# lvclark/tagdigger

Hardware: NVIDIA B200
Metric: reads/sec (whole box), 200M-read 96-plex GBS FASTQ (higher is better)
Workload: dtype u8 text -> 2-bit keys, int32 counts

## Files before the change

### tagdigger_b200/csrc/tdg_kernel.cuh

```cuda
#pragma once
#include <cuda_runtime.h>
#include <stdint.h>
#include <stddef.h>
#include "tdg_match.h"

namespace tdg {

#ifndef TDG_WARPS
#define TDG_WARPS 14
#endif
#ifndef TDG_CHUNKS
#define TDG_CHUNKS 15
#endif
#ifndef TDG_HALO
#define TDG_HALO 256
#endif

constexpr int      WARPS = TDG_WARPS;
constexpr int      THREADS = WARPS * 32;
constexpr uint32_t CHUNKS = TDG_CHUNKS;
constexpr uint32_t SPAN = CHUNKS * 16;
constexpr uint32_t MWORDS = (SPAN + 31) / 32;
constexpr uint32_t HALF_WORDS = MWORDS / 2;
constexpr uint32_t TILE = 32 * SPAN;
// ... 73 lines not shown
    unsigned long long *totals;
};

struct VerifyArgs {
    uint32_t num_segs;
    uint32_t use_arg_state;
    uint32_t prev_kind;
    uint32_t make_fixes;
    unsigned long long line_base;
    unsigned long long reads_limit;
    const LineState *state_in;
    LineState *state_out;
    const SegInfo *seginfo;
    const uint32_t *last_kind;
    FixEntry *fix;
    uint32_t *n_fix;
    unsigned long long *run_total;
};

inline uint32_t fast_words_for(const BarTable *bar, const TagTable &tt)
{
    if (bar->any_base || tt.any_base) return 0;
    if (bar->max_len > 16 || bar->max_tag_off > 28) return 0;
    if (tt.n_classes != 1 || tt.max_len > 64 + LONG_TAIL_MAX || tt.min_len < 1) return 0;
    uint32_t chars = 3 + bar->max_tag_off + tt.max_len;
    if (chars < 3 + 16) chars = 3 + 16;
    uint32_t nw = (chars + 3) / 4;
    return nw <= (tt.max_len > 64 ? LONG_WORDS_MAX : FAST_WORDS_MAX) ? nw : 0;
}
inline bool fast_is_long(const TagTable &tt) { return tt.max_len > 64; }

#if defined(__CUDACC__)

struct alignas(16) WarpShared {
    uint16_t q[QCAP];
    uint16_t gs[GUESS_LINES + 8];
};
static_assert(sizeof(WarpShared) % 16 == 0, "control blocks must keep the barcode table 16-byte aligned");

constexpr size_t SMEM_FIXED = (size_t)WARPS * RING + (size_t)WARPS * sizeof(WarpShared);

__device__ __forceinline__ uint32_t smem_u32(const void *p)
{
    return (uint32_t)__cvta_generic_to_shared(p);
}
__device__ __forceinline__ void mbar_init(uint64_t *bar, uint32_t count)
{
    asm volatile("mbarrier.init.shared::cta.b64 [%0], %1;" ::"r"(smem_u32(bar)), "r"(count));
}
__device__ __forceinline__ void mbar_expect_tx(uint64_t *bar, uint32_t bytes)
{
    asm volatile("mbarrier.arrive.expect_tx.shared::cta.b64 _, [%0], %1;" ::"r"(smem_u32(bar)), "r"(bytes)
                 : "memory");
}
__device__ __forceinline__ void mbar_wait(uint64_t *bar, uint32_t parity)
{
    asm volatile(
        "{\n"
        ".reg .pred p;\n"
        "WAIT_%=:\n"
        "mbarrier.try_wait.parity.shared::cta.b64 p, [%0], %1;\n"
        "@p bra DONE_%=;\n"
        "bra WAIT_%=;\n"
        "DONE_%=:\n"
        "}\n" ::"r"(smem_u32(bar)),
        "r"(parity)
        : "memory");
}
__device__ __forceinline__ bool mbar_test(uint64_t *bar, uint32_t parity)
{
    uint32_t ok;
    asm volatile(
        "{\n"
        ".reg .pred p;\n"
        "mbarrier.try_wait.parity.shared::cta.b64 p, [%1], %2;\n"
        "selp.u32 %0, 1, 0, p;\n"
        "}\n"
        : "=r"(ok)
        : "r"(smem_u32(bar)), "r"(parity)
        : "memory");
    return ok != 0;
}
__device__ __forceinline__ void bulk_g2s(void *dst, const void *src, uint32_t bytes, uint64_t *bar)
{
    uint64_t policy;
    asm volatile("createpolicy.fractional.L2::evict_first.b64 %0, 1.0;" : "=l"(policy));
    asm volatile(
        "cp.async.bulk.shared::cluster.global.mbarrier::complete_tx::bytes.L2::cache_hint [%0], [%1], %2, [%3], %4;" ::"r"(
            smem_u32(dst)),
        "l"(src), "r"(bytes), "r"(smem_u32(bar)), "l"(policy)
        : "memory");
}

__device__ __forceinline__ uint32_t notctl4(uint32_t w)
{
    uint32_t r;
    asm("prmt.b32 %0, %1, %2, %3;" : "=r"(r) : "r"(w + 0x60606060u), "r"(0u), "r"(0xBA98u));
    return r;
}
__device__ __forceinline__ int32_t dp4a_su(uint32_t a_signed_bytes, uint32_t b_unsigned_bytes, int32_t c)
{
    int32_t d;
    asm("dp4a.s32.u32 %0, %1, %2, %3;" : "=r"(d) : "r"(a_signed_bytes), "r"(b_unsigned_bytes), "r"(c));
    return d;
}
__device__ __forceinline__ uint32_t ctl_mask16(uint4 q, uint32_t &dev)
{
    const uint32_t nx = notctl4(q.x), ny = notctl4(q.y), nz = notctl4(q.z), nw = notctl4(q.w);
    const int32_t lo = dp4a_su(ny, 0x80402010u, dp4a_su(nx, 0x08040201u, 255));
    const int32_t hi = dp4a_su(nw, 0x80402010u, dp4a_su(nz, 0x08040201u, 255));
    dev |= ((q.x ^ 0x0A0A0A0Au) & ~nx) | ((q.y ^ 0x0A0A0A0Au) & ~ny);
    dev |= ((q.z ^ 0x0A0A0A0Au) & ~nz) | ((q.w ^ 0x0A0A0A0Au) & ~nw);
    return (uint32_t)hi * 256u + (uint32_t)lo;
}

struct SmemFetch {
    const uint8_t *p;
    uint32_t limit;
    __device__ __forceinline__ void load8(uint32_t off, uint32_t w[8]) const
    {
        const uint8_t *q = p + off;
        uint32_t sh = ((uint32_t)(uintptr_t)q & 3u) * 8u;
        const uint32_t *a = (const uint32_t *)((uintptr_t)q & ~(uintptr_t)3);
        uint32_t prev = a[0];
#pragma unroll
        for (int i = 0; i < 8; i++) {
            uint32_t nxt = a[i + 1];
            w[i] = __funnelshift_r(prev, nxt, sh);
            prev = nxt;
        }
    }
};

struct GlobalFetch {
    const uint8_t *p;
    uint32_t limit;
    __device__ __forceinline__ void load8(uint32_t off, uint32_t w[8]) const
    {
#pragma unroll 1
        for (int i = 0; i < 8; i++) {
            uint32_t v = 0;
            for (int k = 0; k < 4; k++) {
                uint32_t o = off + 4 * i + k;
                uint32_t c = o < limit ? p[o] : 0u;
                v |= c << (8 * k);
            }
            w[i] = v;
        }
    }
};

__device__ __noinline__ MatchResult match_general(const uint8_t *buf, uint32_t pos, uint32_t staged,
                                                  const uint8_t *gtile, unsigned long long avail, uint32_t need,
                                                  const BarTable *bar, const BarEntry *bent, const TagTable *tt)
{
    while (pos < staged) {
        uint32_t c = buf[pos];
        if (is_lead_space(c)) { pos++; continue; }
        if (c >= 0xC2 && c <= 0xE3 && pos + 2 < staged) {
            uint32_t u = utf8_space(c, buf[pos + 1], buf[pos + 2]);
            if (u) { pos += u; continue; }
        }
        break;
    }
    if (pos + need <= staged || staged == avail) {
        SmemFetch f;
        f.p = buf + pos;
        unsigned long long room = avail - pos;
        f.limit = room > 0x7FFFFFFFull ? 0x7FFFFFFFu : (uint32_t)room;
        return match_line(f, bar, bent, *tt);
    }
    unsigned long long gp = pos;
    while (gp < avail) {
        uint32_t c = gtile[gp];
        if (is_lead_space(c)) { gp++; continue; }
        if (c >= 0xC2 && c <= 0xE3 && gp + 2 < avail) {
            uint32_t u = utf8_space(c, gtile[gp + 1], gtile[gp + 2]);
            if (u) { gp += u; continue; }
        }
        break;
    }
    GlobalFetch f;
    f.p = gtile + gp;
    unsigned long long room = avail - gp;
    f.limit = room > 0x7FFFFFFFull ? 0x7FFFFFFFu : (uint32_t)room;
    return match_line(f, bar, bent, *tt);
}

__device__ __forceinline__ uint32_t pack_word(uint32_t w, uint32_t &bad)
{
    uint32_t c2 = (w >> 1) & 0x03030303u;
    uint32_t m = (c2 >> 1) & ~c2 & 0x01010101u;
    bad = (w & 0xD9D9D9D9u) ^ (0x41414141u ^ (m * 0x11u));
    return c2 * 0x01041040u;
}

__device__ __forceinline__ uint32_t lowmask32(uint32_t nbases)
{
    return nbases >= 16 ? 0xFFFFFFFFu : ((1u << (2 * nbases)) - 1u);
}

template <bool MATCH, bool LONG = false>
__global__ void __launch_bounds__(THREADS, 1) count_kernel(const __grid_constant__ ChunkArgs a)
{
    extern __shared__ __align__(128) uint8_t smem[];
    __shared__ __align__(8) uint64_t full_bar[WARPS][STAGES];

    constexpr uint32_t NONE = 0xFFFFFFFFu;
    constexpr uint32_t FULL = 0xFFFFFFFFu;
    const uint32_t tid = threadIdx.x;
    const uint32_t lane = tid & 31u;
    const uint32_t warp = tid >> 5;

    uint8_t *const wbase = smem + (size_t)warp * RING;
    WarpShared *const ws = (WarpShared *)(smem + (size_t)WARPS * RING) + warp;
    uint8_t *const bar_smem = smem + SMEM_FIXED;

    const uint32_t prev_kind = a.use_arg_state ? a.prev_kind : a.state_in->prev_kind;
    if ((a.mode == MODE_FIX ? *a.n_fix : a.num_segs) == 0) return;

    const BarTable *bar = a.bar;
    if (MATCH) {
        if (a.bar_in_smem) {
            const uint4 *src = (const uint4 *)a.bar;
            uint4 *dst = (uint4 *)bar_smem;
            for (uint32_t i = tid; i < (a.bar_bytes + 15u) / 16u; i += THREADS) dst[i] = src[i];
            bar = (const BarTable *)bar_smem;
        }
    }
    const BarEntry *bent = (const BarEntry *)((const uint8_t *)bar + sizeof(BarTable));
    if (lane == 0) {
        for (int s = 0; s < STAGES; s++) mbar_init(&full_bar[warp][s], 1);
        asm volatile("fence.mbarrier_init.release.cluster;" ::: "memory");
        asm volatile("fence.proxy.async.shared::cta;" ::: "memory");
    }
    __syncthreads();

    const uint32_t copy_bytes = TILE + a.halo_bytes;

    uint32_t p_item = NONE, p_seg = 0, p_tix = 0, p_ntiles = 0;
    uint32_t ticket = 0;
    if (lane == 0) ticket = atomicAdd((unsigned int *)a.ticket, 1u);
    auto produce = [&](uint32_t st, uint32_t &m_tile, uint32_t &m_item, uint32_t &m_tixf) {
        if (p_tix == p_ntiles) {
            const uint32_t n_items = a.mode == MODE_FIX ? 2u * *a.n_fix : a.num_segs;
            const uint32_t t = __shfl_sync(FULL, ticket, 0);
            p_tix = 0;
            if (t < n_items) {
                p_item = t;
                const uint32_t seg = a.mode == MODE_FIX ? a.fix[t >> 1].seg : t;
                const bool big = seg < a.n_big;
                const uint32_t want = big ? a.seg_tiles : a.seg_small;
                p_seg = big ? seg * a.seg_tiles : a.n_big * a.seg_tiles + (seg - a.n_big) * a.seg_small;
                const uint32_t left = a.num_tiles - p_seg;
                p_ntiles = left < want ? left : want;
            } else {
                p_item = NONE;
                p_ntiles = NONE;
            }
            asm volatile("" ::"r"(p_item), "r"(p_seg), "r"(p_ntiles));
        }
        m_tile = p_seg + p_tix;
        m_item = p_item;
        m_tixf = p_tix + 1 == p_ntiles ? (p_tix | TIX_LAST) : p_tix;
        if (p_item != NONE) {
            if (lane == 0) {
                const unsigned long long off = (unsigned long long)m_tile * TILE;
                uint32_t bytes = copy_bytes;
                if (__builtin_expect(m_tile + 2 >= a.num_tiles, 0)) {
                    const unsigned long long left = a.n - off;
                    if (left < bytes) bytes = ((uint32_t)left + 15u) & ~15u;
                }
                mbar_expect_tx(&full_bar[warp][st], bytes);
                bulk_g2s(wbase + st * STAGE, a.bytes + off, bytes, &full_bar[warp][st]);
            }
            p_tix++;
            if (p_tix == p_ntiles && lane == 0) ticket = atomicAdd((unsigned int *)a.ticket, 1u);
        }
    };

    const uint32_t nw = MATCH ? a.fast_words : 0;
    int32_t *wmatrix = a.matrix;
    if (MATCH && a.n_replicas > 1) {
        const uint32_t rep = (blockIdx.x * WARPS + warp) % a.n_replicas;
        if (rep) wmatrix = a.replicas + (size_t)(rep - 1) * a.cells;
    }
    const uint4 *tag_entries = (const uint4 *)a.tags.entries;
    int32_t my_bar = 0, my_tag = 0;

    uint32_t seg_lines = 0;
    uint32_t seg_reads = 0;
    uint32_t phase = 0;
    bool has_limit = false;
    int32_t weight = 1;
    bool need_guess = false;
    bool classify_first = false;

    uint32_t cur_tile = 0, cur_item = NONE, cur_tixf = 0;
    uint32_t nxt_tile[STAGES - 1], nxt_item[STAGES - 1], nxt_tixf[STAGES - 1];

    auto tag_differs = [&](const uint4 &k, uint32_t L, uint32_t T0, uint32_t T1, uint32_t T2, uint32_t T3) -> uint32_t {
        if (a.ulen) return ((k.x ^ T0) & a.um[0]) | ((k.y ^ T1) & a.um[1]) | ((k.z ^ T2) & a.um[2]) | ((k.w ^ T3) & a.um[3]);
        return ((k.x ^ T0) & lowmask32(L)) | ((k.y ^ T1) & lowmask32(L > 16 ? L - 16 : 0)) |
               ((k.z ^ T2) & lowmask32(L > 32 ? L - 32 : 0)) | ((k.w ^ T3) & lowmask32(L > 48 ? L - 48 : 0));
    };

    bool pb_pending = false;
    int32_t pb_row = -1, pb_col = -1;
    bool pb_probe = false;
    uint32_t pb_T0 = 0, pb_T1 = 0, pb_T2 = 0, pb_T3 = 0, pb_h = 0, pb_V = 0xFFFFFFFFu, pb_end = 0;
    uint4 pb_k0 = make_uint4(0, 0, 0, 0), pb_k1 = pb_k0;
    uint2 pb_m0 = make_uint2(0, 0), pb_m1 = pb_m0;
    uint32_t pb_x0 = 0, pb_x1 = 0;
    uint32_t pb_TL[LONG ? LONG_TAIL_MAX / 16 : 1];
    constexpr uint32_t NG = (LONG ? LONG_WORDS_MAX : FAST_WORDS_MAX) / 4;

    auto batch_front = [&](uint32_t qoff, uint32_t nb, uint32_t st) {
        uint32_t off = st * STAGE;
        const bool have = lane < nb;
        if (have) off = ws->q[qoff + lane];
        pb_row = -1;
        pb_col = -1;
        pb_probe = false;
        const uint32_t c0 = (*(const uint32_t *)(wbase + (off & ~3u)) >> (8u * (off & 3u))) & 0xFFu;
        const bool lead = (c0 == 0x09) | (c0 == 0x0b) | (c0 == 0x0c) | ((c0 - 0x1cu) <= 4u) | (c0 >= 0x80);
        const bool slow = have & ((nw == 0) | (cur_tile + 2 >= a.num_tiles) | lead);
        __syncwarp();
        if (nw != 0) {
            const uint32_t sh = off & 3u;
            const uint32_t *wp = (const uint32_t *)(wbase + (off & ~3u));
            uint32_t P[NG + 1];
            uint32_t GB[NG];
            auto pack_group = [&](uint32_t g) {
                uint32_t x[4], gbad = 0;
#pragma unroll
                for (uint32_t k = 0; k < 4; k++) {
                    uint32_t bad;
                    x[k] = pack_word(wp[4 * g + k], bad);
                    if (g == 0 && k == 0) bad &= 0xFFFFFFFFu << (8u * sh);
                    gbad |= bad;
                }
                GB[g] = gbad;
                P[g] = __byte_perm(__byte_perm(x[0], x[1], 0x0073), __byte_perm(x[2], x[3], 0x0073), 0x5410);
            };
#pragma unroll
            for (uint32_t g = 0; g < NG; g++) { P[g] = 0; GB[g] = 0; }
            P[NG] = 0;
            pack_group(0);
            pack_group(1);
            const uint32_t key0 = __funnelshift_r(P[0], P[1], 2u * sh);
            uint32_t tag_off = 0, blen = 0;
            int32_t row = -1;
            {
                const uint32_t b = key0 & 0xFFu;
                const uint32_t lo = bar->bucket[b], hi = bar->bucket[b + 1];
                const uint4 be0 = *(const uint4 *)(bent + lo), be1 = *(const uint4 *)(bent + lo + 1);
                const bool h0 = (lo < hi) & (((key0 ^ be0.x) & be0.y) == 0);
                const bool h1 = (lo + 1 < hi) & (((key0 ^ be1.x) & be1.y) == 0);
                uint32_t rz = h0 ? be0.z : be1.z, rw = h0 ? be0.w : be1.w;
                bool hit = h0 | h1;
                if (!hit & (lo + 2 < hi)) {
                    for (uint32_t e = lo + 2; e < hi; e++) {
                        const uint4 be = *(const uint4 *)(bent + e);
                        if (((key0 ^ be.x) & be.y) == 0) { rz = be.z; rw = be.w; hit = true; break; }
                    }
                }
                if (hit) {
                    row = (int32_t)rz;
                    blen = rw & 0xFFFFu;
                    tag_off = rw >> 16;
                }
            }
            __syncwarp();
            pack_group(2);
            pack_group(3);
            const uint32_t toff = sh + tag_off;
            const uint32_t bit = (toff & 15u) * 2u;
            const bool up = (toff >> 4) != 0;
            {
                const uint32_t Q0 = up ? P[1] : P[0], Q1 = up ? P[2] : P[1], Q2 = up ? P[3] : P[2];
                pb_T0 = __funnelshift_r(Q0, Q1, bit);
                pb_T1 = __funnelshift_r(Q1, Q2, bit);
            }
            const uint64_t pre = (((uint64_t)pb_T1 << 32) | pb_T0) & a.tag_km;
            pb_h = tag_slot(pre, a.tags.cls[0].mask);
            const bool want = have & !slow & (row >= 0);
            {
                const uint4 *e0 = tag_entries + 2 * (size_t)(a.tags.cls[0].base + (want ? pb_h : 0u));
                pb_k0 = __ldg(e0);
                if (LONG) {
                    const uint4 f0 = __ldg(e0 + 1), f1 = __ldg(e0 + 3);
                    pb_m0 = make_uint2(f0.x, f0.y);
                    pb_m1 = make_uint2(f1.x, f1.y);
                    pb_x0 = f0.z;
                    pb_x1 = f1.z;
                } else {
                    pb_m0 = __ldg((const uint2 *)(e0 + 1));
                    pb_m1 = __ldg((const uint2 *)(e0 + 3));
                }
                pb_k1 = __ldg(e0 + 2);
            }
#pragma unroll
            for (uint32_t g = 4; g < NG; g++)
                if (nw > 4 * g) pack_group(g);
            {
                const uint32_t Q2 = up ? P[3] : P[2], Q3 = up ? P[4] : P[3], Q4 = up ? P[5] : P[4];
                pb_T2 = __funnelshift_r(Q2, Q3, bit);
                pb_T3 = __funnelshift_r(Q3, Q4, bit);
            }
            if (LONG) {
#pragma unroll
                for (uint32_t j = 0; j < LONG_TAIL_MAX / 16; j++) {
                    const uint32_t Qa = up ? P[5 + j] : P[4 + j], Qb = up ? P[6 + j] : P[5 + j];
                    pb_TL[j] = __funnelshift_r(Qa, Qb, bit);
                }
            }
            uint32_t V = 0xFFFFFFFFu;
            uint32_t anybad = 0;
#pragma unroll
            for (uint32_t g = 0; g < NG; g++) anybad |= GB[g];
            if (anybad != 0) {
                uint32_t i0 = 0;
#pragma unroll
                for (int g = (int)NG - 1; g >= 0; g--)
                    if (GB[g] != 0) i0 = 4u * g;
                const uint32_t Vmin = i0 ? 4u * i0 - sh : 0u, Vmax = 4u * i0 + 15u - sh;
                const uint32_t end_max = tag_off + a.tags.max_len, end_min = tag_off + a.tags.min_len;
                const bool bar_amb = (blen > Vmin) & (blen <= Vmax);
                const bool tag_amb = (blen <= Vmin) & (end_max > Vmin) & (end_min <= Vmax);
                V = Vmin;
                if (want & (bar_amb | tag_amb)) {
                    uint32_t firstbad = 0, at = 0;
#pragma unroll
                    for (int k = 3; k >= 0; k--) {
                        uint32_t bad;
                        (void)pack_word(wp[i0 + k], bad);
                        if (i0 + k == 0) bad &= 0xFFFFFFFFu << (8u * sh);
                        if (bad != 0 && i0 + k < nw) { firstbad = bad; at = i0 + k; }
                    }
                    V = firstbad ? 4u * at + ((uint32_t)(__ffs(firstbad) - 1) >> 3) - sh : 0xFFFFFFFFu;
                }
            }
            __syncwarp();
            pb_probe = want & (blen <= V);
            if (pb_probe) {
                pb_row = row;
                pb_V = V;
                pb_end = tag_off;
            }
        }
        if (slow) {
            const uint32_t p = off - st * STAGE;
            const unsigned long long tile_off = (unsigned long long)cur_tile * TILE;
            const unsigned long long avail = a.n - tile_off;
            const uint32_t staged = avail < copy_bytes ? (uint32_t)avail : copy_bytes;
            MatchResult mr = match_general(wbase + st * STAGE, p, staged, a.bytes + tile_off, avail, a.need, bar, bent, &a.tags);
            pb_row = mr.row;
            pb_col = mr.col;
        }
        __syncwarp();
        pb_pending = true;
    };

    uint32_t pr_cell = NONE, pr_peers = 0;
    auto red_retire = [&]() {
        if (pr_cell != NONE && lane == (uint32_t)(__ffs(pr_peers) - 1))
            asm volatile("red.global.add.s32 [%0], %1;" ::"l"(wmatrix + pr_cell), "r"(weight * (int32_t)__popc(pr_peers)) : "memory");
        pr_cell = NONE;
    };

    auto batch_back = [&]() {
        red_retire();
        {
            const bool e0 = pb_m0.x == TDG_EMPTY_LEN, e1 = pb_m1.x == TDG_EMPTY_LEN;
            const uint32_t L0 = pb_m0.x & TDG_LEN_MASK;
            bool hit0 = !e0 & (tag_differs(pb_k0, L0, pb_T0, pb_T1, pb_T2, pb_T3) == 0);
            bool hit1 = !e0 & !e1 & (LONG | !hit0) & (tag_differs(pb_k1, pb_m1.x, pb_T0, pb_T1, pb_T2, pb_T3) == 0);
            if (LONG) {
                const uint64_t *x0 = a.tags.ext + ((hit0 & pb_probe & (L0 > 64u)) ? pb_x0 : 0u);
                const uint64_t *x1 = a.tags.ext + ((hit1 & pb_probe & (pb_m1.x > 64u)) ? pb_x1 : 0u);
                uint2 t0[LONG_TAIL_MAX / 32], t1[LONG_TAIL_MAX / 32];
#pragma unroll
                for (uint32_t j = 0; j < LONG_TAIL_MAX / 32; j++) {
                    t0[j] = __ldg((const uint2 *)(x0 + j));
                    t1[j] = __ldg((const uint2 *)(x1 + j));
                }
                auto tail_differs = [&](const uint2 (&t)[LONG_TAIL_MAX / 32], uint32_t L) -> uint32_t {
                    const uint32_t rest = L > 64u ? L - 64u : 0u;
                    uint32_t d = 0;
#pragma unroll
                    for (uint32_t j = 0; j < LONG_TAIL_MAX / 32; j++) {
                        d |= (t[j].x ^ pb_TL[2 * j]) & lowmask32(rest > 32u * j ? rest - 32u * j : 0u);
                        d |= (t[j].y ^ pb_TL[2 * j + 1]) & lowmask32(rest > 32u * j + 16u ? rest - 32u * j - 16u : 0u);
                    }
                    return d;
                };
                hit0 = hit0 & (tail_differs(t0, L0) == 0);
                hit1 = hit1 & !hit0 & (tail_differs(t1, pb_m1.x) == 0);
            }
            int32_t col = hit0 ? (int32_t)pb_m0.y : (hit1 ? (int32_t)pb_m1.y : -1);
            uint32_t tlen = hit0 ? L0 : pb_m1.x;
            auto long_tail_ok = [&](const uint4 *half, uint32_t L) -> bool {
                if (L <= 64u) return true;
                const uint64_t *x = a.tags.ext + __ldg(half).z;
                const uint32_t rest = L - 64u;
                uint32_t d = 0;
#pragma unroll
                for (uint32_t j = 0; j < LONG_TAIL_MAX / 32; j++) {
                    const uint2 t = __ldg((const uint2 *)(x + j));
                    d |= (t.x ^ pb_TL[LONG ? 2 * j : 0]) & lowmask32(rest > 32u * j ? rest - 32u * j : 0u);
                    d |= (t.y ^ pb_TL[LONG ? 2 * j + 1 : 0]) & lowmask32(rest > 32u * j + 16u ? rest - 32u * j - 16u : 0u);
                }
                return d == 0;
            };
            if (pb_probe & !e0 & !e1 & !hit0 & !hit1 & ((pb_m0.x & TDG_LEN_MORE) != 0)) {
                uint32_t h = pb_h;
                for (;;) {
                    h = (h + 2) & a.tags.cls[0].mask;
                    const uint4 *e = tag_entries + 2 * (size_t)(a.tags.cls[0].base + h);
                    const uint4 k0 = __ldg(e), k1 = __ldg(e + 2);
                    const uint2 m0 = __ldg((const uint2 *)(e + 1)), m1 = __ldg((const uint2 *)(e + 3));
                    if (m0.x == TDG_EMPTY_LEN) break;
                    const uint32_t l0 = m0.x & TDG_LEN_MASK;
                    if (tag_differs(k0, l0, pb_T0, pb_T1, pb_T2, pb_T3) == 0 && (!LONG || long_tail_ok(e + 1, l0))) {
                        col = (int32_t)m0.y; tlen = l0; break;
                    }
                    if (m1.x == TDG_EMPTY_LEN) break;
                    if (tag_differs(k1, m1.x, pb_T0, pb_T1, pb_T2, pb_T3) == 0 && (!LONG || long_tail_ok(e + 3, m1.x))) {
                        col = (int32_t)m1.y; tlen = m1.x; break;
                    }
                    if (!(m0.x & TDG_LEN_MORE)) break;
                }
            }
            __syncwarp();
            if (pb_probe) pb_col = (col >= 0 && pb_end + tlen > pb_V) ? -1 : col;
        }
        if (pb_row >= 0) my_bar += weight;
        uint32_t cell = NONE;
        if (pb_col >= 0) {
            my_tag += weight;
            cell = (uint32_t)pb_row * a.cols + (uint32_t)pb_col;
        }
        pr_cell = cell;
        pr_peers = __match_any_sync(FULL, cell);
        pb_pending = false;
    };

    uint32_t s = 0, parity = 0;
    uint32_t mk[MWORDS];
#pragma unroll
    for (uint32_t j = 0; j < MWORDS; j++) mk[j] = 0;
    uint32_t scan_dev = 0;
    bool opened = false;

    produce(0, cur_tile, cur_item, cur_tixf);
#pragma unroll
    for (int k = 0; k < STAGES - 1; k++) produce(k + 1, nxt_tile[k], nxt_item[k], nxt_tixf[k]);

    for (;;) {
        if (opened) {
            const uint8_t *const buf = wbase + s * STAGE;
            const uint32_t sbase = s * STAGE;
            const uint32_t t = cur_tile;
            const bool seg_end = (cur_tixf & TIX_LAST) != 0;
            const bool edge = (t == 0) | (t + 2 >= a.num_tiles);
            uint32_t avail = 0xFFFFFFFFu;
            uint32_t extra = 0;
            if (edge) {
                if (t + 2 >= a.num_tiles) {
                    const unsigned long long avail64 = a.n - (unsigned long long)t * TILE;
                    avail = avail64 > 0xFFFFFFFFull ? 0xFFFFFFFFu : (uint32_t)avail64;
                }
                if (t == 0) {
                    if (prev_kind == PREV_NONE || prev_kind == PREV_LF) extra = 1;
                    else if (prev_kind == PREV_CR && buf[0] != '\n') extra = 1;
                }
            }
            if (classify_first | __any_sync(FULL, scan_dev != 0)) {
                classify_first = true;
#pragma unroll
                for (uint32_t j = 0; j < MWORDS; j++) {
                    uint32_t m = mk[j], keepm = m;
                    while (m) {
                        const uint32_t b = __ffs(m) - 1u;
                        m &= m - 1u;
                        const uint32_t p = lane * SPAN + 32 * j + b;
                        const uint32_t c = buf[p];
                        bool end = c == '\n';
                        if (c == '\r') end = (p + 1 < avail) && buf[p + 1] != '\n';
                        if (!end) keepm &= ~(1u << b);
                    }
                    mk[j] = keepm;
                }
                __syncwarp();
            }
            uint32_t cntA = 0, cntB = 0;
#pragma unroll
            for (uint32_t j = 0; j < MWORDS; j++) {
                if (j < HALF_WORDS) cntA += __popc(mk[j]); else cntB += __popc(mk[j]);
            }
            const uint32_t cnt = cntA + cntB;

            uint32_t incl, total;
            if (!__any_sync(FULL, cnt >= 8u)) {
                const uint32_t upto = 0xFFFFFFFFu >> (31u - lane);
                const uint32_t b0 = __ballot_sync(FULL, (cnt & 1u) != 0), b1 = __ballot_sync(FULL, (cnt & 2u) != 0),
                               b2 = __ballot_sync(FULL, (cnt & 4u) != 0);
                incl = __popc(b0 & upto) + 2u * __popc(b1 & upto) + 4u * __popc(b2 & upto);
                total = extra + __popc(b0) + 2u * __popc(b1) + 4u * __popc(b2);
            } else {
                incl = cnt;
#pragma unroll
                for (int d = 1; d < 32; d <<= 1) {
                    uint32_t o = __shfl_up_sync(FULL, incl, d);
                    if (lane >= (uint32_t)d) incl += o;
                }
                total = extra + __shfl_sync(FULL, incl, 31);
            }
            uint32_t nlive = 0;
            if (MATCH) {
                const uint32_t rhoA = extra + incl - cnt;
                if (need_guess) {
                    if (rhoA < GUESS_LINES + 5) {
                        uint32_t r = rhoA;
#pragma unroll
                        for (uint32_t j = 0; j < MWORDS; j++) {
                            uint32_t m = mk[j];
                            while (m && r < GUESS_LINES + 5) {
                                const uint32_t b = __ffs(m) - 1u;
                                m &= m - 1u;
                                ws->gs[r] = (uint16_t)(lane * SPAN + 32 * j + b + 1);
                                r++;
                            }
                        }
                    }
                    __syncwarp();
                    const uint32_t have = total < GUESS_LINES + 5 ? total : GUESS_LINES + 5;
                    bool hit = false;
                    if (lane < GUESS_LINES && lane + 4 < have) {
                        uint32_t p0 = ws->gs[lane], p1 = ws->gs[lane + 1], p2 = ws->gs[lane + 2], p3 = ws->gs[lane + 3],
                                 p4 = ws->gs[lane + 4];
                        hit = buf[p0] == '@' && buf[p2] == '+' && p2 - p1 == p4 - p3;
                    }
                    const uint32_t hits = __ballot_sync(FULL, hit);
                    phase = hits ? ((4u - ((uint32_t)(__ffs(hits) - 1) & 3u)) & 3u) : 0u;
                    need_guess = false;
                }
                const uint32_t a4 = (1u - (phase + seg_lines)) & 3u;
                const uint32_t nq = total > a4 ? (total - a4 + 3u) >> 2 : 0u;
                nlive = nq;
                if (has_limit) {
                    const unsigned long long seg_first = a.fix[cur_item >> 1].true_first;
                    const unsigned long long first_idx = (seg_first + seg_lines + a4) >> 2;
                    nlive = 0;
                    if (nq && first_idx < a.reads_limit) {
                        unsigned long long room = a.reads_limit - first_idx;
                        nlive = nq < room ? nq : (uint32_t)room;
                    }
                }
                const uint32_t rhoB = rhoA + cntA;
                const uint32_t skipA = (a4 - rhoA) & 3u, skipB = (a4 - rhoB) & 3u;
                const bool fast = !(edge | has_limit | (nq > QCAP)) &&
                                  !__any_sync(FULL, (cntA > skipA + 4u) | (cntB > skipB + 4u));
                if (fast) {
                    uint32_t mA = 0, pA = 0, rA = skipA, seen = 0;
#pragma unroll
                    for (uint32_t j = 0; j < HALF_WORDS; j++) {
                        const uint32_t w = mk[j];
                        if (skipA >= seen) { mA = w; pA = 32u * j; rA = skipA - seen; }
                        seen += __popc(w);
                    }
                    uint32_t mB = 0, pB = 0, rB = skipB;
                    seen = 0;
#pragma unroll
                    for (uint32_t j = HALF_WORDS; j < MWORDS; j++) {
                        const uint32_t w = mk[j];
                        if (skipB >= seen) { mB = w; pB = 32u * j; rB = skipB - seen; }
                        seen += __popc(w);
                    }
                    if (rA >= 1u) mA &= mA - 1u;
                    if (rA >= 2u) mA &= mA - 1u;
                    if (rA >= 3u) mA &= mA - 1u;
                    if (rB >= 1u) mB &= mB - 1u;
                    if (rB >= 2u) mB &= mB - 1u;
                    if (rB >= 3u) mB &= mB - 1u;
                    const uint32_t mine = sbase + lane * SPAN;
                    if (cntA > skipA) ws->q[(rhoA + skipA - a4) >> 2] = (uint16_t)(mine + pA + __ffs(mA));
                    if (cntB > skipB) ws->q[(rhoB + skipB - a4) >> 2] = (uint16_t)(mine + pB + __ffs(mB));
                }
                for (uint32_t w0 = 0; w0 < nlive;) {
                    const uint32_t room = nlive - w0 < 32u ? nlive - w0 : 32u;
                    if (!fast) {
                        const uint32_t skip0 = skipA, jj0 = (rhoA + skipA - a4) >> 2;
                        uint32_t skip = skip0, jj = jj0;
#pragma unroll
                        for (uint32_t j = 0; j < MWORDS; j++) {
                            uint32_t m = mk[j];
                            while (m) {
                                const uint32_t b = __ffs(m) - 1u;
                                m &= m - 1u;
                                if (skip == 0) {
                                    if (jj - w0 < room) ws->q[jj - w0] = (uint16_t)(sbase + lane * SPAN + 32 * j + b + 1);
                                    jj++;
                                    skip = 3;
                                } else {
                                    skip--;
                                }
                            }
                        }
                        if (extra != 0 && lane == 0 && a4 == 0 && w0 == 0) ws->q[0] = (uint16_t)sbase;
                    }
                    __syncwarp();
                    if (pb_pending) batch_back();
                    batch_front(fast ? w0 : 0u, room, s);
                    w0 += room;
                    if (w0 >= nlive) break;
                }
            }
            seg_lines += total;
            seg_reads += nlive;

            if (seg_end) {
                if (MATCH) {
                    if (pb_pending) batch_back();
                    red_retire();
                }
                if (lane == 0) {
                    if (MATCH && seg_reads) atomicAdd(&a.totals[0], (unsigned long long)(weight * (long long)seg_reads));
                    if (a.mode == MODE_MAIN) {
                        SegInfo si;
                        si.lines = seg_lines;
                        si.guess = phase;
                        a.seginfo[cur_item] = si;
                    }
                }
                seg_reads = 0;
            }

            __syncwarp();
            if (lane == 0) asm volatile("fence.proxy.async.shared::cta;" ::: "memory");
            cur_tile = nxt_tile[0];
            cur_item = nxt_item[0];
            cur_tixf = nxt_tixf[0];
#pragma unroll
            for (int k = 0; k + 1 < STAGES - 1; k++) {
                nxt_tile[k] = nxt_tile[k + 1];
                nxt_item[k] = nxt_item[k + 1];
                nxt_tixf[k] = nxt_tixf[k + 1];
            }
            produce(s, nxt_tile[STAGES - 2], nxt_item[STAGES - 2], nxt_tixf[STAGES - 2]);
            if (++s == STAGES) { s = 0; parity ^= 1u; }
        }

        if (cur_item == NONE) break;
        if (!mbar_test(&full_bar[warp][s], parity)) mbar_wait(&full_bar[warp][s], parity);

        if ((cur_tixf & ~TIX_LAST) == 0) {
            seg_lines = 0;
            has_limit = false;
            weight = 1;
            need_guess = false;
            if (a.mode == MODE_FIX) {
                const FixEntry fe = a.fix[cur_item >> 1];
                if (cur_item & 1u) { phase = (uint32_t)fe.true_first & 3u; has_limit = true; }
                else               { phase = fe.guess & 3u; weight = -1; }
            } else if (cur_item == 0) {
                phase = (uint32_t)(a.use_arg_state ? a.line_base : a.state_in->next_line) & 3u;
            } else {
                phase = 0;
                need_guess = MATCH;
            }
            asm volatile("" ::"r"(phase));
        }

        {
            const uint4 *src = (const uint4 *)(wbase + s * STAGE + lane * SPAN);
            scan_dev = 0;
#pragma unroll
            for (uint32_t i = 0; i < CHUNKS; i++) {
                if (MATCH && i == (CHUNKS + 1) / 2) {
                    if (pb_pending) batch_back();
                }
                uint32_t m16 = ctl_mask16(src[i], scan_dev);
                if (i & 1u) mk[i >> 1] |= m16 << 16; else mk[i >> 1] = m16;
            }
        }
        if (cur_tile == a.num_tiles - 1) {
            const unsigned long long avail64 = a.n - (unsigned long long)cur_tile * TILE;
            const uint32_t valid = avail64 < TILE ? (uint32_t)avail64 : TILE;
            const uint32_t lim = valid - 1;
            const uint32_t first = lane * SPAN;
            const uint32_t keep = lim > first ? lim - first : 0;
#pragma unroll
            for (uint32_t j = 0; j < MWORDS; j++) {
                uint32_t nb = keep > 32 * j ? keep - 32 * j : 0;
                if (nb < 32) mk[j] &= (1u << nb) - 1u;
            }
            if (lane == 0) {
                uint32_t c = (wbase + s * STAGE)[valid - 1];
                *a.last_kind = c == '\n' ? PREV_LF : (c == '\r' ? PREV_CR : PREV_OTHER);
            }
        }
        if (MATCH) red_retire();
        opened = true;
    }

    if (MATCH) {
#pragma unroll
        for (int o = 16; o > 0; o >>= 1) {
            my_bar += __shfl_xor_sync(FULL, my_bar, o);
            my_tag += __shfl_xor_sync(FULL, my_tag, o);
        }
    }
    if (lane == 0) {
        if (MATCH) {
            if (my_bar) atomicAdd(&a.totals[1], (unsigned long long)(long long)my_bar);
            if (my_tag) atomicAdd(&a.totals[2], (unsigned long long)(long long)my_tag);
        }
    }
}

__global__ void __launch_bounds__(256) fold_kernel(int32_t *matrix, int32_t *replicas, uint32_t cells, uint32_t extra)
{
    for (uint32_t i = blockIdx.x * blockDim.x + threadIdx.x; i < cells; i += gridDim.x * blockDim.x) {
        int32_t sum = 0;
        for (uint32_t r = 0; r < extra; r++) {
            int32_t v = replicas[(size_t)r * cells + i];
            if (v) { sum += v; replicas[(size_t)r * cells + i] = 0; }
        }
        if (sum) matrix[i] += sum;
    }
}

__global__ void __launch_bounds__(256) min_kernel(const int32_t *matrix, uint32_t cells, int32_t *out)
{
    int32_t m = 0x7FFFFFFF;
    for (uint32_t i = blockIdx.x * blockDim.x + threadIdx.x; i < cells; i += gridDim.x * blockDim.x) {
        const int32_t v = matrix[i];
        m = v < m ? v : m;
    }
#pragma unroll
    for (int o = 16; o > 0; o >>= 1) {
        const int32_t v = __shfl_xor_sync(0xFFFFFFFFu, m, o);
        m = v < m ? v : m;
    }
    if ((threadIdx.x & 31u) == 0) atomicMin(out, m);
}

constexpr int VERIFY_THREADS = 1024;
constexpr uint32_t VERIFY_MAX_CTAS = 32;
__device__ __forceinline__ void verify_run(const VerifyArgs &v, uint32_t &lo, uint32_t &hi)
{
    const uint32_t nruns = gridDim.x * (VERIFY_THREADS / 32);
    const uint32_t run = blockIdx.x * (VERIFY_THREADS / 32) + (threadIdx.x >> 5);
    const uint32_t per = ((v.num_segs + nruns - 1) / nruns + 31u) & ~31u;
    lo = (unsigned long long)run * per < v.num_segs ? run * per : v.num_segs;
    hi = (unsigned long long)lo + per < v.num_segs ? lo + per : v.num_segs;
}

__global__ void __launch_bounds__(VERIFY_THREADS) verify_sums(const VerifyArgs v)
{
    const uint32_t lane = threadIdx.x & 31u;
    uint32_t lo, hi;
    verify_run(v, lo, hi);
    unsigned long long sum = 0;
    for (uint32_t i = lo + lane; i < hi; i += 128) {
        uint32_t part[4];
#pragma unroll
        for (uint32_t k = 0; k < 4; k++) part[k] = i + 32 * k < hi ? __ldg(&v.seginfo[i + 32 * k].lines) : 0u;
        sum += (unsigned long long)part[0] + part[1] + part[2] + part[3];
    }
#pragma unroll
    for (int o = 16; o > 0; o >>= 1) sum += __shfl_xor_sync(0xFFFFFFFFu, sum, o);
    if (lane == 0) v.run_total[blockIdx.x * (VERIFY_THREADS / 32) + (threadIdx.x >> 5)] = sum;
}

__global__ void __launch_bounds__(VERIFY_THREADS) verify_kernel(const VerifyArgs v)
{
    const uint32_t tid = threadIdx.x, lane = tid & 31u;
    const unsigned long long line_base = v.use_arg_state ? v.line_base : v.state_in->next_line;
    const uint32_t nruns = gridDim.x * (VERIFY_THREADS / 32);
    const uint32_t run = blockIdx.x * (VERIFY_THREADS / 32) + (tid >> 5);
    uint32_t lo, hi;
    verify_run(v, lo, hi);

    unsigned long long before = 0, total = 0;
    for (uint32_t w = lane; w < nruns; w += 32) {
        const unsigned long long t = v.run_total[w];
        if (w < run) before += t;
        total += t;
    }
#pragma unroll
    for (int o = 16; o > 0; o >>= 1) {
        before += __shfl_xor_sync(0xFFFFFFFFu, before, o);
        total += __shfl_xor_sync(0xFFFFFFFFu, total, o);
    }

    if (v.make_fixes) {
        unsigned long long first = line_base + before;
        for (uint32_t i0 = lo; i0 < hi; i0 += 128) {
            uint2 part[4];
#pragma unroll
            for (uint32_t k = 0; k < 4; k++) {
                const uint32_t i = i0 + 32 * k + lane;
                part[k] = i < hi ? __ldg((const uint2 *)&v.seginfo[i]) : make_uint2(0u, 0u);
            }
#pragma unroll
            for (uint32_t k = 0; k < 4; k++) {
                const uint32_t i = i0 + 32 * k + lane;
                const uint32_t lines = part[k].x, guess = part[k].y;
                uint32_t incl = lines;
#pragma unroll
                for (int d = 1; d < 32; d <<= 1) {
                    const uint32_t o = __shfl_up_sync(0xFFFFFFFFu, incl, d);
                    if (lane >= (uint32_t)d) incl += o;
                }
                const unsigned long long mine = first + (incl - lines);
                const bool wrong = ((mine ^ guess) & 3ull) != 0;
                const bool past = lines && ((mine + lines - 1) >> 2) >= v.reads_limit;
                if (lines && (wrong || past)) {
                    const uint32_t slot = atomicAdd(v.n_fix, 1u);
                    FixEntry fe;
                    fe.seg = i;
                    fe.guess = guess;
                    fe.true_first = mine;
                    v.fix[slot] = fe;
                }
                first += __shfl_sync(0xFFFFFFFFu, incl, 31);
            }
        }
    }
    if (blockIdx.x == 0 && tid == 0) {
        v.state_out->next_line = line_base + total;
        v.state_out->prev_kind = *v.last_kind;
        v.state_out->pad = 0;
    }
}

#endif

}
```

Baseline: 20.43 billion.

## Restructure per-tile loop into a flat state machine overlapping batch matching with scans

Flattens the per-tile inner batch loop into the outer loop. Each iteration now issues at most one 32-read batch_front, and batch_back is interleaved between the two halves of the control-character scan. The weight is carried with the pending batch so it can be retired after a segment boundary. Warp shuffles and ballots are replaced by __reduce_*_sync intrinsics, and branch hints are added on rare paths. The intent is to hide match latency behind the scan and to cut warp divergence and loop overhead, at the cost of a more complex control flow that must also drain pending batches at segment ends and on exit.

Result: no change. 20.63 billion, median of 6 (+1.0%).

```diff
diff --git a/tagdigger_b200/csrc/tdg_kernel.cuh b/tagdigger_b200/csrc/tdg_kernel.cuh
--- a/tagdigger_b200/csrc/tdg_kernel.cuh
+++ b/tagdigger_b200/csrc/tdg_kernel.cuh
@@ -249,8 +249,9 @@
 
 __device__ __noinline__ MatchResult match_general(const uint8_t *buf, uint32_t pos, uint32_t staged,
                                                   const uint8_t *gtile, unsigned long long avail, uint32_t need,
-                                                  const BarTable *bar, const BarEntry *bent, const TagTable *tt)
-{
+                                                  const BarTable *bar, const TagTable *tt)
+{
+    const BarEntry *bent = (const BarEntry *)((const uint8_t *)bar + sizeof(BarTable));
     while (pos < staged) {
         uint32_t c = buf[pos];
         if (is_lead_space(c)) { pos++; continue; }
@@ -340,12 +341,12 @@
     if (lane == 0) ticket = atomicAdd((unsigned int *)a.ticket, 1u);
     auto produce = [&](uint32_t st, uint32_t &m_tile, uint32_t &m_item, uint32_t &m_tixf) {
         if (p_tix == p_ntiles) {
-            const uint32_t n_items = a.mode == MODE_FIX ? 2u * *a.n_fix : a.num_segs;
-            const uint32_t t = __shfl_sync(FULL, ticket, 0);
+            const uint32_t n_items = a.mode == MODE_FIX ? 2u * __reduce_or_sync(FULL, *a.n_fix) : a.num_segs;
+            const uint32_t t = __reduce_or_sync(FULL, ticket);
             p_tix = 0;
             if (t < n_items) {
                 p_item = t;
-                const uint32_t seg = a.mode == MODE_FIX ? a.fix[t >> 1].seg : t;
+                const uint32_t seg = a.mode == MODE_FIX ? __reduce_or_sync(FULL, a.fix[t >> 1].seg) : t;
                 const bool big = seg < a.n_big;
                 const uint32_t want = big ? a.seg_tiles : a.seg_small;
                 p_seg = big ? seg * a.seg_tiles : a.n_big * a.seg_tiles + (seg - a.n_big) * a.seg_small;
@@ -403,6 +404,7 @@
     };
 
     bool pb_pending = false;
+    int32_t pb_w = 1;
     int32_t pb_row = -1, pb_col = -1;
     bool pb_probe = false;
     uint32_t pb_T0 = 0, pb_T1 = 0, pb_T2 = 0, pb_T3 = 0, pb_h = 0, pb_V = 0xFFFFFFFFu, pb_end = 0;
@@ -551,18 +553,19 @@
             const unsigned long long tile_off = (unsigned long long)cur_tile * TILE;
             const unsigned long long avail = a.n - tile_off;
             const uint32_t staged = avail < copy_bytes ? (uint32_t)avail : copy_bytes;
-            MatchResult mr = match_general(wbase + st * STAGE, p, staged, a.bytes + tile_off, avail, a.need, bar, bent, &a.tags);
+            MatchResult mr = match_general(wbase + st * STAGE, p, staged, a.bytes + tile_off, avail, a.need, bar, &a.tags);
             pb_row = mr.row;
             pb_col = mr.col;
         }
         __syncwarp();
         pb_pending = true;
+        pb_w = weight;
     };
 
     uint32_t pr_cell = NONE, pr_peers = 0;
     auto red_retire = [&]() {
         if (pr_cell != NONE && lane == (uint32_t)(__ffs(pr_peers) - 1))
-            asm volatile("red.global.add.s32 [%0], %1;" ::"l"(wmatrix + pr_cell), "r"(weight * (int32_t)__popc(pr_peers)) : "memory");
+            asm volatile("red.global.add.s32 [%0], %1;" ::"l"(wmatrix + pr_cell), "r"(pb_w * (int32_t)__popc(pr_peers)) : "memory");
         pr_cell = NONE;
     };
 
@@ -632,10 +635,10 @@
             __syncwarp();
             if (pb_probe) pb_col = (col >= 0 && pb_end + tlen > pb_V) ? -1 : col;
         }
-        if (pb_row >= 0) my_bar += weight;
+        if (pb_row >= 0) my_bar += pb_w;
         uint32_t cell = NONE;
         if (pb_col >= 0) {
-            my_tag += weight;
+            my_tag += pb_w;
             cell = (uint32_t)pb_row * a.cols + (uint32_t)pb_col;
         }
         pr_cell = cell;
@@ -649,6 +652,10 @@
     for (uint32_t j = 0; j < MWORDS; j++) mk[j] = 0;
     uint32_t scan_dev = 0;
     bool opened = false;
+    bool more = false;
+    uint32_t w0 = 0;
+    uint32_t total = 0, nlive = 0;
+    bool fast = false;
 
     produce(0, cur_tile, cur_item, cur_tixf);
 #pragma unroll
@@ -656,138 +663,139 @@
 
     for (;;) {
         if (opened) {
-            const uint8_t *const buf = wbase + s * STAGE;
-            const uint32_t sbase = s * STAGE;
-            const uint32_t t = cur_tile;
-            const bool seg_end = (cur_tixf & TIX_LAST) != 0;
-            const bool edge = (t == 0) | (t + 2 >= a.num_tiles);
-            uint32_t avail = 0xFFFFFFFFu;
-            uint32_t extra = 0;
-            if (edge) {
-                if (t + 2 >= a.num_tiles) {
-                    const unsigned long long avail64 = a.n - (unsigned long long)t * TILE;
-                    avail = avail64 > 0xFFFFFFFFull ? 0xFFFFFFFFu : (uint32_t)avail64;
-                }
-                if (t == 0) {
-                    if (prev_kind == PREV_NONE || prev_kind == PREV_LF) extra = 1;
-                    else if (prev_kind == PREV_CR && buf[0] != '\n') extra = 1;
-                }
-            }
-            if (classify_first | __any_sync(FULL, scan_dev != 0)) {
-                classify_first = true;
-#pragma unroll
+            if (!(more & fast)) {
+                const uint8_t *const buf = wbase + s * STAGE;
+                const uint32_t sbase = s * STAGE;
+                const uint32_t t = cur_tile;
+                const bool edge = (t == 0) | (t + 2 >= a.num_tiles);
+                uint32_t avail = 0xFFFFFFFFu;
+                uint32_t extra = 0;
+                if (__builtin_expect(edge, 0)) {
+                    if (t + 2 >= a.num_tiles) {
+                        const unsigned long long avail64 = a.n - (unsigned long long)t * TILE;
+                        avail = avail64 > 0xFFFFFFFFull ? 0xFFFFFFFFu : (uint32_t)avail64;
+                    }
+                    if (t == 0) {
+                        if (prev_kind == PREV_NONE || prev_kind == PREV_LF) extra = 1;
+                        else if (prev_kind == PREV_CR && buf[0] != '\n') extra = 1;
+                    }
+                }
+                if (__builtin_expect(classify_first | __any_sync(FULL, scan_dev != 0), 0)) {
+                    classify_first = true;
+    #pragma unroll
+                    for (uint32_t j = 0; j < MWORDS; j++) {
+                        uint32_t m = mk[j], keepm = m;
+                        while (m) {
+                            const uint32_t b = __ffs(m) - 1u;
+                            m &= m - 1u;
+                            const uint32_t p = lane * SPAN + 32 * j + b;
+                            const uint32_t c = buf[p];
+                            bool end = c == '\n';
+                            if (c == '\r') end = (p + 1 < avail) && buf[p + 1] != '\n';
+                            if (!end) keepm &= ~(1u << b);
+                        }
+                        mk[j] = keepm;
+                    }
+                    __syncwarp();
+                }
+                uint32_t cntA = 0, cntB = 0;
+    #pragma unroll
                 for (uint32_t j = 0; j < MWORDS; j++) {
-                    uint32_t m = mk[j], keepm = m;
-                    while (m) {
-                        const uint32_t b = __ffs(m) - 1u;
-                        m &= m - 1u;
-                        const uint32_t p = lane * SPAN + 32 * j + b;
-                        const uint32_t c = buf[p];
-                        bool end = c == '\n';
-                        if (c == '\r') end = (p + 1 < avail) && buf[p + 1] != '\n';
-                        if (!end) keepm &= ~(1u << b);
-                    }
-                    mk[j] = keepm;
-                }
-                __syncwarp();
-            }
-            uint32_t cntA = 0, cntB = 0;
-#pragma unroll
-            for (uint32_t j = 0; j < MWORDS; j++) {
-                if (j < HALF_WORDS) cntA += __popc(mk[j]); else cntB += __popc(mk[j]);
-            }
-            const uint32_t cnt = cntA + cntB;
-
-            uint32_t incl, total;
-            if (!__any_sync(FULL, cnt >= 8u)) {
-                const uint32_t upto = 0xFFFFFFFFu >> (31u - lane);
-                const uint32_t b0 = __ballot_sync(FULL, (cnt & 1u) != 0), b1 = __ballot_sync(FULL, (cnt & 2u) != 0),
-                               b2 = __ballot_sync(FULL, (cnt & 4u) != 0);
-                incl = __popc(b0 & upto) + 2u * __popc(b1 & upto) + 4u * __popc(b2 & upto);
-                total = extra + __popc(b0) + 2u * __popc(b1) + 4u * __popc(b2);
-            } else {
-                incl = cnt;
-#pragma unroll
-                for (int d = 1; d < 32; d <<= 1) {
-                    uint32_t o = __shfl_up_sync(FULL, incl, d);
-                    if (lane >= (uint32_t)d) incl += o;
-                }
-                total = extra + __shfl_sync(FULL, incl, 31);
-            }
-            uint32_t nlive = 0;
-            if (MATCH) {
-                const uint32_t rhoA = extra + incl - cnt;
-                if (need_guess) {
-                    if (rhoA < GUESS_LINES + 5) {
-                        uint32_t r = rhoA;
-#pragma unroll
-                        for (uint32_t j = 0; j < MWORDS; j++) {
-                            uint32_t m = mk[j];
-                            while (m && r < GUESS_LINES + 5) {
-                                const uint32_t b = __ffs(m) - 1u;
-                                m &= m - 1u;
-                                ws->gs[r] = (uint16_t)(lane * SPAN + 32 * j + b + 1);
-                                r++;
+                    if (j < HALF_WORDS) cntA += __popc(mk[j]); else cntB += __popc(mk[j]);
+                }
+                const uint32_t cnt = cntA + cntB;
+
+                total = __reduce_add_sync(FULL, cnt + (lane == 0 ? extra : 0u));
+                uint32_t incl;
+                if (!__any_sync(FULL, cnt >= 8u)) {
+                    const uint32_t upto = 0xFFFFFFFFu >> (31u - lane);
+                    const uint32_t b0 = __ballot_sync(FULL, (cnt & 1u) != 0), b1 = __ballot_sync(FULL, (cnt & 2u) != 0),
+                                   b2 = __ballot_sync(FULL, (cnt & 4u) != 0);
+                    incl = __popc(b0 & upto) + 2u * __popc(b1 & upto) + 4u * __popc(b2 & upto);
+                } else {
+                    incl = cnt;
+    #pragma unroll
+                    for (int d = 1; d < 32; d <<= 1) {
+                        uint32_t o = __shfl_up_sync(FULL, incl, d);
+                        if (lane >= (uint32_t)d) incl += o;
+                    }
+                }
+                nlive = 0;
+                if (MATCH) {
+                    const uint32_t rhoA = extra + incl - cnt;
+                    if (__builtin_expect(need_guess, 0)) {
+                        if (rhoA < GUESS_LINES + 5) {
+                            uint32_t r = rhoA;
+    #pragma unroll
+                            for (uint32_t j = 0; j < MWORDS; j++) {
+                                uint32_t m = mk[j];
+                                while (m && r < GUESS_LINES + 5) {
+                                    const uint32_t b = __ffs(m) - 1u;
+                                    m &= m - 1u;
+                                    ws->gs[r] = (uint16_t)(lane * SPAN + 32 * j + b + 1);
+                                    r++;
+                                }
                             }
                         }
-                    }
-                    __syncwarp();
-                    const uint32_t have = total < GUESS_LINES + 5 ? total : GUESS_LINES + 5;
-                    bool hit = false;
-                    if (lane < GUESS_LINES && lane + 4 < have) {
-                        uint32_t p0 = ws->gs[lane], p1 = ws->gs[lane + 1], p2 = ws->gs[lane + 2], p3 = ws->gs[lane + 3],
-                                 p4 = ws->gs[lane + 4];
-                        hit = buf[p0] == '@' && buf[p2] == '+' && p2 - p1 == p4 - p3;
-                    }
-                    const uint32_t hits = __ballot_sync(FULL, hit);
-                    phase = hits ? ((4u - ((uint32_t)(__ffs(hits) - 1) & 3u)) & 3u) : 0u;
-                    need_guess = false;
-                }
-                const uint32_t a4 = (1u - (phase + seg_lines)) & 3u;
-                const uint32_t nq = total > a4 ? (total - a4 + 3u) >> 2 : 0u;
-                nlive = nq;
-                if (has_limit) {
-                    const unsigned long long seg_first = a.fix[cur_item >> 1].true_first;
-                    const unsigned long long first_idx = (seg_first + seg_lines + a4) >> 2;
-                    nlive = 0;
-                    if (nq && first_idx < a.reads_limit) {
-                        unsigned long long room = a.reads_limit - first_idx;
-                        nlive = nq < room ? nq : (uint32_t)room;
-                    }
-                }
-                const uint32_t rhoB = rhoA + cntA;
-                const uint32_t skipA = (a4 - rhoA) & 3u, skipB = (a4 - rhoB) & 3u;
-                const bool fast = !(edge | has_limit | (nq > QCAP)) &&
-                                  !__any_sync(FULL, (cntA > skipA + 4u) | (cntB > skipB + 4u));
-                if (fast) {
-                    uint32_t mA = 0, pA = 0, rA = skipA, seen = 0;
-#pragma unroll
-                    for (uint32_t j = 0; j < HALF_WORDS; j++) {
-                        const uint32_t w = mk[j];
-                        if (skipA >= seen) { mA = w; pA = 32u * j; rA = skipA - seen; }
-                        seen += __popc(w);
-                    }
-                    uint32_t mB = 0, pB = 0, rB = skipB;
-                    seen = 0;
-#pragma unroll
-                    for (uint32_t j = HALF_WORDS; j < MWORDS; j++) {
-                        const uint32_t w = mk[j];
-                        if (skipB >= seen) { mB = w; pB = 32u * j; rB = skipB - seen; }
-                        seen += __popc(w);
-                    }
-                    if (rA >= 1u) mA &= mA - 1u;
-                    if (rA >= 2u) mA &= mA - 1u;
-                    if (rA >= 3u) mA &= mA - 1u;
-                    if (rB >= 1u) mB &= mB - 1u;
-                    if (rB >= 2u) mB &= mB - 1u;
-                    if (rB >= 3u) mB &= mB - 1u;
-                    const uint32_t mine = sbase + lane * SPAN;
-                    if (cntA > skipA) ws->q[(rhoA + skipA - a4) >> 2] = (uint16_t)(mine + pA + __ffs(mA));
-                    if (cntB > skipB) ws->q[(rhoB + skipB - a4) >> 2] = (uint16_t)(mine + pB + __ffs(mB));
-                }
-                for (uint32_t w0 = 0; w0 < nlive;) {
-                    const uint32_t room = nlive - w0 < 32u ? nlive - w0 : 32u;
-                    if (!fast) {
+                        __syncwarp();
+                        const uint32_t have = total < GUESS_LINES + 5 ? total : GUESS_LINES + 5;
+                        bool hit = false;
+                        if (lane < GUESS_LINES && lane + 4 < have) {
+                            uint32_t p0 = ws->gs[lane], p1 = ws->gs[lane + 1], p2 = ws->gs[lane + 2], p3 = ws->gs[lane + 3],
+                                     p4 = ws->gs[lane + 4];
+                            hit = buf[p0] == '@' && buf[p2] == '+' && p2 - p1 == p4 - p3;
+                        }
+                        const uint32_t first = __reduce_min_sync(FULL, hit ? lane : 32u);
+                        phase = first < 32u ? (4u - (first & 3u)) & 3u : 0u;
+                        need_guess = false;
+                    }
+                    const uint32_t a4 = (1u - (phase + seg_lines)) & 3u;
+                    const uint32_t nq = total > a4 ? (total - a4 + 3u) >> 2 : 0u;
+                    nlive = nq;
+                    if (__builtin_expect(has_limit, 0)) {
+                        const unsigned long long true_first = a.fix[cur_item >> 1].true_first;
+                        const unsigned long long seg_first =
+                            ((unsigned long long)__reduce_or_sync(FULL, (uint32_t)(true_first >> 32)) << 32) |
+                            __reduce_or_sync(FULL, (uint32_t)true_first);
+                        const unsigned long long first_idx = (seg_first + seg_lines + a4) >> 2;
+                        nlive = 0;
+                        if (nq && first_idx < a.reads_limit) {
+                            unsigned long long room = a.reads_limit - first_idx;
+                            nlive = nq < room ? nq : (uint32_t)room;
+                        }
+                    }
+                    const uint32_t rhoB = rhoA + cntA;
+                    const uint32_t skipA = (a4 - rhoA) & 3u, skipB = (a4 - rhoB) & 3u;
+                    fast = !(edge | has_limit | (nq > QCAP)) &&
+                                      !__any_sync(FULL, (cntA > skipA + 4u) | (cntB > skipB + 4u));
+                    if (fast) {
+                        uint32_t mA = 0, pA = 0, rA = skipA, seen = 0;
+    #pragma unroll
+                        for (uint32_t j = 0; j < HALF_WORDS; j++) {
+                            const uint32_t w = mk[j];
+                            if (skipA >= seen) { mA = w; pA = 32u * j; rA = skipA - seen; }
+                            seen += __popc(w);
+                        }
+                        uint32_t mB = 0, pB = 0, rB = skipB;
+                        seen = 0;
+    #pragma unroll
+                        for (uint32_t j = HALF_WORDS; j < MWORDS; j++) {
+                            const uint32_t w = mk[j];
+                            if (skipB >= seen) { mB = w; pB = 32u * j; rB = skipB - seen; }
+                            seen += __popc(w);
+                        }
+                        if (rA >= 1u) mA &= mA - 1u;
+                        if (rA >= 2u) mA &= mA - 1u;
+                        if (rA >= 3u) mA &= mA - 1u;
+                        if (rB >= 1u) mB &= mB - 1u;
+                        if (rB >= 2u) mB &= mB - 1u;
+                        if (rB >= 3u) mB &= mB - 1u;
+                        const uint32_t mine = sbase + lane * SPAN;
+                        if (cntA > skipA) ws->q[(rhoA + skipA - a4) >> 2] = (uint16_t)(mine + pA + __ffs(mA));
+                        if (cntB > skipB) ws->q[(rhoB + skipB - a4) >> 2] = (uint16_t)(mine + pB + __ffs(mB));
+                    }
+                    if (__builtin_expect(!fast, 0) && w0 < nlive) {
+                        const uint32_t room = nlive - w0 < 32u ? nlive - w0 : 32u;
                         const uint32_t skip0 = skipA, jj0 = (rhoA + skipA - a4) >> 2;
                         uint32_t skip = skip0, jj = jj0;
 #pragma unroll
@@ -807,98 +815,116 @@
                         }
                         if (extra != 0 && lane == 0 && a4 == 0 && w0 == 0) ws->q[0] = (uint16_t)sbase;
                     }
-                    __syncwarp();
-                    if (pb_pending) batch_back();
-                    batch_front(fast ? w0 : 0u, room, s);
-                    w0 += room;
-                    if (w0 >= nlive) break;
-                }
-            }
-            seg_lines += total;
-            seg_reads += nlive;
-
-            if (seg_end) {
-                if (MATCH) {
-                    if (pb_pending) batch_back();
-                    red_retire();
-                }
-                if (lane == 0) {
-                    if (MATCH && seg_reads) atomicAdd(&a.totals[0], (unsigned long long)(weight * (long long)seg_reads));
-                    if (a.mode == MODE_MAIN) {
-                        SegInfo si;
-                        si.lines = seg_lines;
-                        si.guess = phase;
-                        a.seginfo[cur_item] = si;
-                    }
-                }
-                seg_reads = 0;
-            }
-
-            __syncwarp();
-            if (lane == 0) asm volatile("fence.proxy.async.shared::cta;" ::: "memory");
-            cur_tile = nxt_tile[0];
-            cur_item = nxt_item[0];
-            cur_tixf = nxt_tixf[0];
-#pragma unroll
-            for (int k = 0; k + 1 < STAGES - 1; k++) {
-                nxt_tile[k] = nxt_tile[k + 1];
-                nxt_item[k] = nxt_item[k + 1];
-                nxt_tixf[k] = nxt_tixf[k + 1];
-            }
-            produce(s, nxt_tile[STAGES - 2], nxt_item[STAGES - 2], nxt_tixf[STAGES - 2]);
-            if (++s == STAGES) { s = 0; parity ^= 1u; }
-        }
-
-        if (cur_item == NONE) break;
-        if (!mbar_test(&full_bar[warp][s], parity)) mbar_wait(&full_bar[warp][s], parity);
-
-        if ((cur_tixf & ~TIX_LAST) == 0) {
-            seg_lines = 0;
-            has_limit = false;
-            weight = 1;
-            need_guess = false;
-            if (a.mode == MODE_FIX) {
-                const FixEntry fe = a.fix[cur_item >> 1];
-                if (cur_item & 1u) { phase = (uint32_t)fe.true_first & 3u; has_limit = true; }
-                else               { phase = fe.guess & 3u; weight = -1; }
-            } else if (cur_item == 0) {
-                phase = (uint32_t)(a.use_arg_state ? a.line_base : a.state_in->next_line) & 3u;
-            } else {
-                phase = 0;
-                need_guess = MATCH;
-            }
-            asm volatile("" ::"r"(phase));
+                }
+            }
+            if (MATCH && w0 < nlive) {
+                const uint32_t room = nlive - w0 < 32u ? nlive - w0 : 32u;
+                __syncwarp();
+                batch_front(fast ? w0 : 0u, room, s);
+                w0 += room;
+            }
+            more = w0 < nlive;
+
+            if (!more) {
+                w0 = 0;
+                seg_lines += total;
+                seg_reads += nlive;
+
+                if (cur_tixf & TIX_LAST) {
+                    if (lane == 0) {
+                        if (MATCH && seg_reads) atomicAdd(&a.totals[0], (unsigned long long)(weight * (long long)seg_reads));
+                        if (a.mode == MODE_MAIN) {
+                            SegInfo si;
+                            si.lines = seg_lines;
+                            si.guess = phase;
+                            a.seginfo[cur_item] = si;
+                        }
+                    }
+                    seg_reads = 0;
+                }
+
+                __syncwarp();
+                if (lane == 0) asm volatile("fence.proxy.async.shared::cta;" ::: "memory");
+                cur_tile = nxt_tile[0];
+                cur_item = nxt_item[0];
+                cur_tixf = nxt_tixf[0];
+#pragma unroll
+                for (int k = 0; k + 1 < STAGES - 1; k++) {
+                    nxt_tile[k] = nxt_tile[k + 1];
+                    nxt_item[k] = nxt_item[k + 1];
+                    nxt_tixf[k] = nxt_tixf[k + 1];
+                }
+                produce(s, nxt_tile[STAGES - 2], nxt_item[STAGES - 2], nxt_tixf[STAGES - 2]);
+                if (++s == STAGES) { s = 0; parity ^= 1u; }
+            }
+        }
+
+        const bool last = !more & (cur_item == NONE);
+        if (last & !(MATCH && pb_pending)) break;
+        const bool open = !more & !last;
+        if (open) {
+            if (!mbar_test(&full_bar[warp][s], parity)) mbar_wait(&full_bar[warp][s], parity);
+
+            if ((cur_tixf & ~TIX_LAST) == 0) {
+                seg_lines = 0;
+                has_limit = false;
+                weight = 1;
+                need_guess = false;
+                if (a.mode == MODE_FIX) {
+                    const FixEntry fe = a.fix[cur_item >> 1];
+                    phase = __reduce_or_sync(FULL, (cur_item & 1u ? (uint32_t)fe.true_first : fe.guess) & 3u);
+                    if (cur_item & 1u) has_limit = true;
+                    else               weight = -1;
+                } else if (cur_item == 0) {
+                    phase = __reduce_or_sync(FULL, (uint32_t)(a.use_arg_state ? a.line_base : a.state_in->next_line) & 3u);
+                } else {
+                    phase = 0;
+                    need_guess = MATCH;
+                }
+                asm volatile("" ::"r"(phase));
+            }
         }
 
         {
             const uint4 *src = (const uint4 *)(wbase + s * STAGE + lane * SPAN);
-            scan_dev = 0;
-#pragma unroll
-            for (uint32_t i = 0; i < CHUNKS; i++) {
-                if (MATCH && i == (CHUNKS + 1) / 2) {
-                    if (pb_pending) batch_back();
-                }
-                uint32_t m16 = ctl_mask16(src[i], scan_dev);
-                if (i & 1u) mk[i >> 1] |= m16 << 16; else mk[i >> 1] = m16;
-            }
-        }
-        if (cur_tile == a.num_tiles - 1) {
-            const unsigned long long avail64 = a.n - (unsigned long long)cur_tile * TILE;
-            const uint32_t valid = avail64 < TILE ? (uint32_t)avail64 : TILE;
-            const uint32_t lim = valid - 1;
-            const uint32_t first = lane * SPAN;
-            const uint32_t keep = lim > first ? lim - first : 0;
-#pragma unroll
-            for (uint32_t j = 0; j < MWORDS; j++) {
-                uint32_t nb = keep > 32 * j ? keep - 32 * j : 0;
-                if (nb < 32) mk[j] &= (1u << nb) - 1u;
-            }
-            if (lane == 0) {
-                uint32_t c = (wbase + s * STAGE)[valid - 1];
-                *a.last_kind = c == '\n' ? PREV_LF : (c == '\r' ? PREV_CR : PREV_OTHER);
-            }
-        }
-        if (MATCH) red_retire();
+            if (open) {
+                scan_dev = 0;
+#pragma unroll
+                for (uint32_t i = 0; i < (CHUNKS + 1) / 2; i++) {
+                    uint32_t m16 = ctl_mask16(src[i], scan_dev);
+                    if (i & 1u) mk[i >> 1] |= m16 << 16; else mk[i >> 1] = m16;
+                }
+            }
+            if (MATCH && pb_pending) batch_back();
+            if (open) {
+#pragma unroll
+                for (uint32_t i = (CHUNKS + 1) / 2; i < CHUNKS; i++) {
+                    uint32_t m16 = ctl_mask16(src[i], scan_dev);
+                    if (i & 1u) mk[i >> 1] |= m16 << 16; else mk[i >> 1] = m16;
+                }
+                if (__builtin_expect(cur_tile == a.num_tiles - 1, 0)) {
+                    const unsigned long long avail64 = a.n - (unsigned long long)cur_tile * TILE;
+                    const uint32_t valid = avail64 < TILE ? (uint32_t)avail64 : TILE;
+                    const uint32_t lim = valid - 1;
+                    const uint32_t first = lane * SPAN;
+                    const uint32_t keep = lim > first ? lim - first : 0;
+#pragma unroll
+                    for (uint32_t j = 0; j < MWORDS; j++) {
+                        uint32_t nb = keep > 32 * j ? keep - 32 * j : 0;
+                        if (nb < 32) mk[j] &= (1u << nb) - 1u;
+                    }
+                    if (lane == 0) {
+                        uint32_t c = (wbase + s * STAGE)[valid - 1];
+                        *a.last_kind = c == '\n' ? PREV_LF : (c == '\r' ? PREV_CR : PREV_OTHER);
+                    }
+                }
+                if (MATCH) red_retire();
+            }
+        }
+        if (last) {
+            red_retire();
+            break;
+        }
         opened = true;
     }
 
```
